# NVIDIA/nvalchemi-toolkit-ops

Measured on AMD Instinct MI355X. Metric: atom-steps/sec (nlist+D3+PME) on 100k-atom PBC box, higher is better.
Workload: dtype f64 (PME) + f32 (D3)

## Files before the change

### nvalchemi-toolkit-ops_amd/csrc/nlist.hip

```cpp
#include <stdlib.h>

#include "binsort.h"
#include "common.h"

namespace {

#define NL_PRUNE_R 8
#ifndef NL_TILE
#define NL_TILE 1024
#endif
#ifndef NL_TILE_F64
#define NL_TILE_F64 768
#endif
#ifndef NL_TILED_WAVES
#define NL_TILED_WAVES 0
#endif
#ifndef NL_CCHUNK
#define NL_CCHUNK 64
#endif
#define NL_MAXROWS 96
#define NL_MIXED 0x7fffffff
#define NL_TILED_GRID 1536
static int nl_tiled_grid() {
  static const int g = [] { const char* e = getenv("NVALCHEMIOPS_NL_TILED_GRID"); const int v = e ? atoi(e) : 0; return v > 0 ? v : NL_TILED_GRID; }();
  return g;
}
template <class T> struct NlSys {
  T cell[9];
  T inv[9];
  T origin[3];
  int cpd[3];
  int R[3];
  int pbc[3];
  int nrange[3];
  int cell_off;
  int ncells;
  int tiled;
  int prune;
  signed char dxlim[NL_PRUNE_R + 1][NL_PRUNE_R + 1];
};
struct NlGlobal {
  int total_cells; int any_wrap; int use_tiled; int pad1;
  int work[4];
  int done[4];
};

struct NlLayout {
  size_t sys, glob, natoms, keys_in, keys_out, vals_in, vals_out, wrap, swrap, spos, srk, cell_start, bins, total;
  long long cell_cap;
};

inline long long nl_cell_cap(int N, int B) { return 4ll * N + 8ll * B; }

inline int nl_key_bits(long long cap) {
  int bits = 1;
  while ((1ll << bits) <= cap && bits < 31) ++bits;
  return bits;
}

NlLayout nl_layout(int N, int B, int dtype) {
  NlLayout L;
  size_t o = 0;
  const size_t sysz = dtype == MI_F32 ? sizeof(NlSys<float>) : sizeof(NlSys<double>);
  const size_t esz = dtype == MI_F32 ? 4 : 8;
  L.cell_cap = nl_cell_cap(N, B);
  auto take = [&](size_t bytes) { size_t at = o; o += mi_align(bytes); return at; };
  L.sys = take(sysz * (size_t)B);
  L.glob = take(sizeof(NlGlobal));
  L.natoms = take(sizeof(int) * (size_t)B);
  L.keys_in = take(sizeof(int) * (size_t)N);
  L.keys_out = take(sizeof(int) * (size_t)N);
  L.vals_in = take(sizeof(int) * (size_t)N);
  L.vals_out = take(sizeof(int) * (size_t)N);
  L.wrap = take(8 * (size_t)N);
  L.swrap = take(8 * (size_t)N);
  L.spos = take(4 * esz * (size_t)N);
  L.srk = take(sizeof(float) * (size_t)N);
  L.cell_start = take(sizeof(int) * (size_t)(L.cell_cap + 2));
  L.bins = take(sizeof(int) * bs_scratch_ints(L.cell_cap + 2));
  L.total = o;
  return L;
}

__device__ __forceinline__ float4 pack4(float x, float y, float z, int idx) { return make_float4(x, y, z, __int_as_float(idx)); }
__device__ __forceinline__ double4 pack4(double x, double y, double z, int idx) { return make_double4(x, y, z, (double)idx); }
__device__ __forceinline__ int idx_of(const float4& v) { return __float_as_int(v.w); }
__device__ __forceinline__ int idx_of(const double4& v) { return (int)v.w; }

__global__ void nl_count_atoms_kernel(const int* __restrict__ batch_idx, int N, int* __restrict__ natoms) {
  const int i = blockIdx.x * blockDim.x + threadIdx.x;
  const bool in = i < N;
  const int s = in ? batch_idx[i] : -1;
  const int s0 = __shfl(s, 0, MI_WAVE);
  const unsigned long long same = __ballot(in && s == s0);
  if ((threadIdx.x & (MI_WAVE - 1)) == 0 && s0 >= 0) atomicAdd(&natoms[s0], __popcll(same));
  if (in && s != s0) atomicAdd(&natoms[s], 1);
}

template <class T>
__device__ void nl_describe_system(const T* __restrict__ cell, const uint8_t* __restrict__ pbc, const int* __restrict__ natoms, int N, T cutoff,
                                   const T* __restrict__ origin, int s, NlSys<T>& S) {
  for (int k = 0; k < 9; ++k) S.cell[k] = cell[9 * (size_t)s + k];
  for (int k = 0; k < 3; ++k) S.origin[k] = origin ? origin[3 * (size_t)s + k] : T(0);
  inverse3(S.cell, S.inv);
  const T* a = S.cell;
  double det = (double)a[0] * ((double)a[4] * a[8] - (double)a[5] * a[7]) - (double)a[1] * ((double)a[3] * a[8] - (double)a[5] * a[6]) +
               (double)a[2] * ((double)a[3] * a[7] - (double)a[4] * a[6]);
  double vol = fabs(det);
  int ns = natoms ? natoms[s] : N;
  double rc = (double)cutoff;
  double apc = vol > 0 ? (double)ns / vol * rc * rc * rc : 0.0;
#ifndef NL_K2_APC
#define NL_K2_APC 64.0
#endif
  int k = apc < NL_K2_APC ? 1 : (apc < 512.0 ? 2 : 3);
  long long cap = 4ll * ns + 8;
  double face[3];
  for (int d = 0; d < 3; ++d) {
    T col[3] = {S.inv[d], S.inv[3 + d], S.inv[6 + d]};
    T ln = sqrt(col[0] * col[0] + col[1] * col[1] + col[2] * col[2]);
    face[d] = 1.0 / (double)ln;
    S.pbc[d] = pbc[3 * (size_t)s + d] ? 1 : 0;
    double want = face[d] * k / (rc * (1.0 + 2e-6));
    S.cpd[d] = want >= 1048576.0 ? 1048576 : (want >= 1.0 ? (int)want : 1);
    S.nrange[d] = S.pbc[d] ? (int)ceil(ln * cutoff) : 0;
  }
  long long tot = (long long)S.cpd[0] * S.cpd[1] * S.cpd[2];
  while (tot > cap) {
    for (int d = 0; d < 3; ++d) S.cpd[d] = S.cpd[d] / 2 > 1 ? S.cpd[d] / 2 : 1;
    tot = (long long)S.cpd[0] * S.cpd[1] * S.cpd[2];
  }
  for (int d = 0; d < 3; ++d) {
    if (S.cpd[d] == 1 && !S.pbc[d]) S.R[d] = 0;
    else S.R[d] = (int)ceil(rc * S.cpd[d] / face[d] * (1.0 + 1e-6));
  }
  S.ncells = (int)tot;
  S.cell_off = 0;
  S.tiled = ((k >= 2 || apc >= 32.0) && (2 * S.R[1] + 1) * (2 * S.R[2] + 1) <= NL_MAXROWS && (!S.pbc[0] || S.R[0] <= S.cpd[0])) ? 1 : 0;
  const bool ortho = a[1] == T(0) && a[2] == T(0) && a[3] == T(0) && a[5] == T(0) && a[6] == T(0) && a[7] == T(0);
  S.prune = (ortho && S.R[0] <= NL_PRUNE_R && S.R[1] <= NL_PRUNE_R && S.R[2] <= NL_PRUNE_R) ? 1 : 0;
}

template <class T>
__global__ __launch_bounds__(256) void nl_setup_kernel(const T* __restrict__ cell, const uint8_t* __restrict__ pbc, const int* __restrict__ natoms, int N,
                                int B, T cutoff, const T* __restrict__ origin, NlSys<T>* __restrict__ sys, NlGlobal* __restrict__ glob,
                                int table_blocks, int4* __restrict__ zero, long long zero_words, int* __restrict__ pk_flag,
                                int* __restrict__ cn_hdr, float cn_scale) {
  constexpr int NE = (NL_PRUNE_R + 1) * (NL_PRUNE_R + 1);
  if (pk_flag && blockIdx.x == 0 && threadIdx.x == 0) *pk_flag = 0;
  if (cn_hdr && blockIdx.x == 0) {
    if (threadIdx.x == 0) { cn_hdr[0] = 0; cn_hdr[1] = 0; cn_hdr[2] = __float_as_int((float)cutoff); cn_hdr[3] = __float_as_int(cn_scale); }
    if (threadIdx.x < MI_CN_SLOTS) reinterpret_cast<unsigned long long*>(cn_hdr)[MI_CN_SLOT_OFFSET_U64 + threadIdx.x] = 0ull;
  }
  if ((int)blockIdx.x > table_blocks) {
    const long long zb = (long long)blockIdx.x - table_blocks - 1, nzb = (long long)gridDim.x - table_blocks - 1;
    for (long long k = zb * blockDim.x + threadIdx.x; k < zero_words; k += nzb * blockDim.x) zero[k] = make_int4(0, 0, 0, 0);
    return;
  }
  if (blockIdx.x > 0) {
    const int t = ((int)blockIdx.x - 1) * blockDim.x + threadIdx.x;
    if (t >= B * NE) return;
    const int s = t / NE, az = (t - s * NE) / (NL_PRUNE_R + 1), ay = t - s * NE - az * (NL_PRUNE_R + 1);
    NlSys<T> S;
    nl_describe_system<T>(cell, pbc, natoms, N, cutoff, origin, s, S);
    if (!S.prune) return;
    const double rc = (double)cutoff;
    double w[3];
    for (int d = 0; d < 3; ++d) {
      const double ln = fabs((double)S.inv[4 * d]);
      w[d] = (S.pbc[d] && ln > 0.0) ? (1.0 / ln) / S.cpd[d] : 0.0;
    }
    const double gz = (az > 1 ? az - 1 : 0) * w[2], gy = (ay > 1 ? ay - 1 : 0) * w[1];
    const double rem = rc * rc - gz * gz - gy * gy;
    int lim;
    if (rem < -1e-6 * rc * rc) lim = -1;
    else if (w[0] > 0.0) { lim = (int)(sqrt(rem > 0.0 ? rem : 0.0) / w[0] * (1.0 + 1e-6)) + 1; if (lim > S.R[0]) lim = S.R[0]; }
    else lim = S.R[0];
    sys[s].dxlim[az][ay] = (signed char)lim;
    return;
  }
  for (int s = threadIdx.x; s < B; s += blockDim.x) {
    NlSys<T> S;
    nl_describe_system<T>(cell, pbc, natoms, N, cutoff, origin, s, S);
    NlSys<T>* dst = sys + s;
    for (int k = 0; k < 9; ++k) { dst->cell[k] = S.cell[k]; dst->inv[k] = S.inv[k]; }
    for (int k = 0; k < 3; ++k) { dst->origin[k] = S.origin[k]; dst->cpd[k] = S.cpd[k]; dst->R[k] = S.R[k]; dst->pbc[k] = S.pbc[k]; dst->nrange[k] = S.nrange[k]; }
    dst->cell_off = 0; dst->ncells = S.ncells; dst->tiled = S.tiled; dst->prune = S.prune;
  }
  __syncthreads();
  __shared__ int wave_tot[4];
  __shared__ int carry_sh, tiled_sh;
  if (threadIdx.x == 0) { carry_sh = 0; tiled_sh = 1; }
  __syncthreads();
  const int lane = threadIdx.x & (MI_WAVE - 1), wave = threadIdx.x / MI_WAVE;
  for (int s0 = 0; s0 < B; s0 += blockDim.x) {
    const int s = s0 + threadIdx.x;
    const int x = s < B ? sys[s].ncells : 0;
    if (s < B && !sys[s].tiled) tiled_sh = 0;
    int inc = x;
#pragma unroll
    for (int o = 1; o < MI_WAVE; o <<= 1) { const int up = __shfl_up(inc, o, MI_WAVE); if (lane >= o) inc += up; }
    if (lane == MI_WAVE - 1) wave_tot[wave] = inc;
    __syncthreads();
    int woff = carry_sh;
    for (int w = 0; w < 4; ++w) woff += (w < wave) ? wave_tot[w] : 0;
    if (s < B) sys[s].cell_off = woff + inc - x;
    __syncthreads();
    if (threadIdx.x == blockDim.x - 1) carry_sh = woff + inc;
    __syncthreads();
  }
  if (threadIdx.x == 0) {
    glob->total_cells = carry_sh;
    glob->any_wrap = 0;
    glob->use_tiled = tiled_sh;
    for (int k = 0; k < 4; ++k) { glob->work[k] = 0; glob->done[k] = 0; }
  }
}

template <class T>
__global__ void nl_assign_kernel(const T* __restrict__ pos, const int* __restrict__ batch_idx, int N, const NlSys<T>* __restrict__ sys,
                                 int* __restrict__ keys, int* __restrict__ count, short4* __restrict__ wrap, NlGlobal* __restrict__ glob) {
  int i = blockIdx.x * blockDim.x + threadIdx.x;
  const bool in = i < N;
  int key = 0;
  if (in) {
    const int s = batch_idx ? batch_idx[i] : 0;
    const NlSys<T>& S = sys[s];
    T p[3] = {pos[3 * (size_t)i] - S.origin[0], pos[3 * (size_t)i + 1] - S.origin[1], pos[3 * (size_t)i + 2] - S.origin[2]}, frac[3];
    rowvec_mat3(p, S.inv, frac);
    int c[3], w[3];
#pragma unroll
    for (int d = 0; d < 3; ++d) {
      int v = (int)floor(frac[d] * (T)S.cpd[d]);
      if (S.pbc[d]) floor_divmod(v, S.cpd[d], w[d], c[d]);
      else { w[d] = 0; c[d] = v < 0 ? 0 : (v >= S.cpd[d] ? S.cpd[d] - 1 : v); }
    }
    key = S.cell_off + c[0] + S.cpd[0] * (c[1] + S.cpd[1] * c[2]);
    keys[i] = key;
    wrap[i] = make_short4((short)w[0], (short)w[1], (short)w[2], 0);
    if (w[0] | w[1] | w[2]) glob->any_wrap = 1;
  }
  bs_wave_add<false>(count, key, in);
}

struct NlCnBuild { const int* numbers; const float* rcov; int nz; float K; float* srk; unsigned long long* slots; const void* cell; int n_cell; const int* batch_idx; };
template <class T>
__global__ void nl_rank_gather_kernel(const T* __restrict__ pos, const int* __restrict__ ids, const int* __restrict__ keys,
                                      const int* __restrict__ cell_start, const short4* __restrict__ wrap, int N,
                                      typename Vec4<T>::type* __restrict__ spos, short4* __restrict__ swrap, int* __restrict__ keys_sorted,
                                      NlCnBuild C) {
  int p = blockIdx.x * blockDim.x + threadIdx.x;
  unsigned long long h = 0;
  if (p < N) {
    const int i = ids[p];
    const int key = keys[i];
    const int b = cell_start[key], e = cell_start[key + 1];
    int rank = 0;
    for (int q = b; q < e; ++q) rank += ids[q] < i ? 1 : 0;
    const int dst = b + rank;
    const T x = pos[3 * (size_t)i], y = pos[3 * (size_t)i + 1], z = pos[3 * (size_t)i + 2];
    spos[dst] = pack4(x, y, z, i);
    swrap[dst] = wrap[i];
    keys_sorted[dst] = key;
    if (C.srk) {
      const float rk = mi_cn_rk(C.numbers[i], C.nz, C.rcov, C.K);
      C.srk[dst] = rk;
      h = mi_cn_atom_hash<T>(i, C.batch_idx ? C.batch_idx[i] : 0, x, y, z, rk);
    }
  }
  if (C.srk) {
    if (p < C.n_cell) h += mi_cn_cell_hash<T>(p, reinterpret_cast<const T*>(C.cell)[p]);
    if (p == 0) h += mi_cn_scale_hash(C.K);
    mi_cn_slot_add(C.slots, p / MI_WAVE, h);
  }
}

struct NlInt3 { int a, b, c; };

template <bool NT = true>
__device__ __forceinline__ void wave_fill(int* __restrict__ dst, long long begin, long long end, int value, int lane) {
  long long n = end - begin;
  if (n <= 0) return;
  int* p = dst + begin;
  int head = (int)(((16 - ((uintptr_t)p & 15)) & 15) >> 2);
  if (head > n) head = (int)n;
  if (lane < head) p[lane] = value;
  long long body = (n - head) >> 2;
  int4* p4 = reinterpret_cast<int4*>(p + head);
  typedef int nl_i4 __attribute__((ext_vector_type(4)));
  const nl_i4 w4 = {value, value, value, value};
  for (long long t = lane; t < body; t += MI_WAVE) {
    if constexpr (NT) __builtin_nontemporal_store(w4, reinterpret_cast<nl_i4*>(p4 + t));
    else *reinterpret_cast<nl_i4*>(p4 + t) = w4;
  }
  long long done = head + (body << 2);
  if (done + lane < n) p[done + lane] = value;
}

__device__ __noinline__ void nl_prefix_runs(int* run_pre, int n, int lane) {
  int carry = 0;
  if (lane == 0) run_pre[0] = 0;
  for (int r0 = 0; r0 < n; r0 += MI_WAVE) {
    const int r = r0 + lane;
    int inc = r < n ? run_pre[r + 1] : 0;
#pragma unroll
    for (int o = 1; o < MI_WAVE; o <<= 1) { const int up = __shfl_up(inc, o, MI_WAVE); if (lane >= o) inc += up; }
    if (r < n) run_pre[r + 1] = carry + inc;
    carry += __shfl(inc, MI_WAVE - 1, MI_WAVE);
  }
}

__device__ __forceinline__ long long nl_uniform64(long long v) {
  const unsigned lo = __builtin_amdgcn_readfirstlane((unsigned)v), hi = __builtin_amdgcn_readfirstlane((unsigned)((unsigned long long)v >> 32));
  return (long long)(((unsigned long long)hi << 32) | lo);
}

__device__ __forceinline__ float nl_uni(float x) { return __int_as_float(__builtin_amdgcn_readfirstlane(__float_as_int(x))); }
__device__ __forceinline__ double nl_uni(double x) { return __longlong_as_double(nl_uniform64(__double_as_longlong(x))); }

template <class T> struct NlSecond { T rc2; int* nm; int* nsh; int* num; int M; };
struct NlPacked { unsigned* words; int* flag; };
struct NlCn { const float* rk; float* cn; int* flag; float K; };
__device__ __forceinline__ float nl_cn_term(float d2, float rki, float rkj, float K) {
  const float rinv = __builtin_amdgcn_rsqf(d2);
  const float t = fmaf(-(rki + rkj), rinv, K);
  return __builtin_amdgcn_rcpf(1.0f + __builtin_amdgcn_exp2f(t));
}
#define NL_PK_PAD 0xffffffffu
#ifndef NL_PREZERO_SHIFTS
#define NL_PREZERO_SHIFTS 1
#endif
#ifndef NL_PREZERO_NT
#define NL_PREZERO_NT 1
#endif
#define NL_PK_ZERO_SHIFT 0x54000000u
__device__ __forceinline__ unsigned nl_pk_code(int Sx, int Sy, int Sz, bool& bad) {
  const unsigned cx = (unsigned)(Sx + 1), cy = (unsigned)(Sy + 1), cz = (unsigned)(Sz + 1);
  bad = (cx > 2u) | (cy > 2u) | (cz > 2u);
  return ((cx & 3u) << 26) | ((cy & 3u) << 28) | (cz << 30);
}

template <class T>
__device__ __forceinline__ bool nl_pair_hit(T pix, T piy, T piz, int i, T cjx, T cjy, T cjz, int j, int Sx, int Sy, int Sz, const T* cart,
                                            T rc2, bool naive, bool half, int nr0, int nr1, int nr2, T* d2_out = nullptr) {
  T dr0, dr1, dr2;
  bool ok = true;
  if (!naive) {
    dr0 = (cjx - pix) + cart[0];
    dr1 = (cjy - piy) + cart[1];
    dr2 = (cjz - piz) + cart[2];
  } else {
    const bool upper = Sx > 0 || (Sx == 0 && Sy > 0) || (Sx == 0 && Sy == 0 && Sz >= 0);
    if (upper) { dr0 = (cart[0] + cjx) - pix; dr1 = (cart[1] + cjy) - piy; dr2 = (cart[2] + cjz) - piz; }
    else { dr0 = ((-cart[0]) + pix) - cjx; dr1 = ((-cart[1]) + piy) - cjy; dr2 = ((-cart[2]) + piz) - cjz; }
    ok = (Sx <= nr0 && -Sx <= nr0) && (Sy <= nr1 && -Sy <= nr1) && (Sz <= nr2 && -Sz <= nr2);
  }
  const T d2 = dr0 * dr0 + dr1 * dr1 + dr2 * dr2;
  if (d2_out) *d2_out = d2;
  const bool zeroS = (Sx | Sy | Sz) == 0;
  bool hit = ok && (d2 < rc2) && !(j == i && zeroS);
  if (half && hit) {
    const bool pos_shift = Sx > 0 || (Sx == 0 && Sy > 0) || (Sx == 0 && Sy == 0 && Sz > 0);
    hit = pos_shift || (zeroS && j > i);
  }
  return hit;
}

template <class T, int MODE, bool FAST, bool DUAL = false, bool CNF = false>
#if NL_TILED_WAVES > 0
__global__ __launch_bounds__(256) __attribute__((amdgpu_waves_per_eu(NL_TILED_WAVES, NL_TILED_WAVES))) void nl_query_tiled_kernel(
#else
__global__ __launch_bounds__(256) __attribute__((amdgpu_waves_per_eu((CNF && sizeof(T) == 4) ? 5 : 1, (CNF && sizeof(T) == 4) ? 5 : 8))) void nl_query_tiled_kernel(
#endif
    const typename Vec4<T>::type* __restrict__ spos, const short4* __restrict__ swrap, const int* __restrict__ cell_start,
    const NlSys<T>* __restrict__ sys, const NlGlobal* __restrict__ glob, int B, T rc2, int flags, int* __restrict__ nm,
    int* __restrict__ nsh, int* __restrict__ num, int M, int fill_value, const int* __restrict__ ptr, int* __restrict__ list_ij,
    int* __restrict__ list_sh, long long P, NlSecond<T> D, NlPacked K, NlCn CN = NlCn{nullptr, nullptr, nullptr, 0.0f}) {
  static_assert(!DUAL || (MODE == MI_NL_MODE_MATRIX && !FAST), "the dual-cutoff sweep is instantiated for the general matrix kernel only");
  static_assert(!CNF || (MODE == MI_NL_MODE_MATRIX && FAST && !DUAL), "coordination numbers ride with the plain full-list matrix search");
  constexpr int TILE = sizeof(T) == 8 ? NL_TILE_F64 : NL_TILE;
  if (!glob->use_tiled) return;
  if (!DUAL && FAST != ((flags & (MI_NL_HALF_FILL | MI_NL_NAIVE_EXPR)) == 0)) return;
  __shared__ float trk[CNF ? TILE : 1], cen_rk[CNF ? NL_CCHUNK : 1];
  __shared__ double ccn[CNF ? NL_CCHUNK : 1];
  __shared__ int ccnt2[DUAL ? NL_CCHUNK : 1];
  __shared__ T tx[TILE], ty[TILE], tz[TILE];
  __shared__ int tj[TILE];
  __shared__ short tsx[CNF ? 1 : TILE], tsy[CNF ? 1 : TILE], tsz[CNF ? 1 : TILE];
  __shared__ int tsp[CNF ? TILE : 1];
  __shared__ int run_beg[3 * NL_MAXROWS], run_pre[3 * NL_MAXROWS + 1], run_cs[3 * NL_MAXROWS];
  __shared__ int ccnt[NL_CCHUNK];
  __shared__ T cen_x[NL_CCHUNK], cen_y[NL_CCHUNK], cen_z[NL_CCHUNK];
  __shared__ int cen_i[NL_CCHUNK];
  __shared__ short4 cen_w[NL_CCHUNK];
  __shared__ int grp_run[TILE / MI_WAVE];
  __shared__ int grp_shift[TILE / MI_WAVE];
  __shared__ int u_store[CNF ? 1 : 9 * NL_MAXROWS];
  static_assert(sizeof(T) * TILE >= sizeof(int) * 9 * NL_MAXROWS, "the run table must fit the x array of a tile");
  int* const u_beg = CNF ? reinterpret_cast<int*>(tx) : u_store;
  int* const u_len = u_beg + 3 * NL_MAXROWS;
  int* const u_cs = u_beg + 6 * NL_MAXROWS;
  const int tid = threadIdx.x, lane = tid & (MI_WAVE - 1), wave = tid / MI_WAVE;
  const int total_cells = glob->total_cells;
  const bool anyw = glob->any_wrap != 0;
  const bool half = (flags & MI_NL_HALF_FILL) != 0, naive = (flags & MI_NL_NAIVE_EXPR) != 0;
  const unsigned long long lt = (1ull << lane) - 1ull;
  __shared__ int next_cell;
  NlGlobal* gw = const_cast<NlGlobal*>(glob);
  for (;;) {
    __syncthreads();
    if (tid == 0) next_cell = atomicAdd(&gw->work[MODE], 1);
    __syncthreads();
    const int c = next_cell;
    if (c >= total_cells) break;
    const int c_beg = cell_start[c], n_c = cell_start[c + 1] - c_beg;
    if (n_c == 0) continue;
    int s = 0;
    {
      int lo = 0, hi = B - 1;
      while (lo < hi) { const int mid = (lo + hi + 1) >> 1; if (sys[mid].cell_off <= c) lo = mid; else hi = mid - 1; }
      s = lo;
    }
    const NlSys<T>* S = sys + s;
    const int nx = S->cpd[0], ny = S->cpd[1], nz = S->cpd[2];
    const int Rx = S->R[0], Ry = S->R[1], Rz = S->R[2];
    const bool pbx = S->pbc[0] != 0, pby = S->pbc[1] != 0, pbz = S->pbc[2] != 0;
    const int coff = S->cell_off;
    const int nr0 = S->nrange[0], nr1 = S->nrange[1], nr2 = S->nrange[2];
    T cm[9];
#pragma unroll
    for (int k = 0; k < 9; ++k) cm[k] = S->cell[k];
    const int local = c - coff;
    const int cx = local % nx, cyz = local / nx, cy = cyz % ny, cz = cyz / ny;
    const int nyr = 2 * Ry + 1, nrows = (2 * Rz + 1) * nyr;
    __syncthreads();
    if (tid < nrows) {
      const int dzr = tid / nyr, dz = dzr - Rz, dy = tid - dzr * nyr - Ry;
      const int tzc = cz + dz, tyc = cy + dy;
      bool ok = (pbz || (tzc >= 0 && tzc < nz)) && (pby || (tyc >= 0 && tyc < ny));
      int csz = 0, wz = tzc, csy = 0, wy = tyc;
      if (ok) {
        while (wz < 0) { wz += nz; --csz; }
        while (wz >= nz) { wz -= nz; ++csz; }
        while (wy < 0) { wy += ny; --csy; }
        while (wy >= ny) { wy -= ny; ++csy; }
      }
      int dxm = Rx;
      if (S->prune) { dxm = S->dxlim[dz < 0 ? -dz : dz][dy < 0 ? -dy : dy]; ok = ok && dxm >= 0; }
      int xlo = cx - dxm, xhi = cx + dxm;
      if (!pbx) { xlo = xlo < 0 ? 0 : xlo; xhi = xhi > nx - 1 ? nx - 1 : xhi; }
      const int rowbase = coff + nx * (wy + ny * wz);
      for (int g = 0; g < 3; ++g) {
        const int img0 = (g - 1) * nx;
        const int xa = (xlo > img0 ? xlo : img0), xb = (xhi < img0 + nx - 1 ? xhi : img0 + nx - 1);
        int b = 0, len = 0;
        if (ok && xa <= xb && (pbx || g == 1)) { b = cell_start[rowbase + xa - img0]; len = cell_start[rowbase + xb - img0 + 1] - b; }
        u_beg[3 * tid + g] = b;
        u_len[3 * tid + g] = len;
        u_cs[3 * tid + g] = ((g - 1) & 0x3ff) | ((csy & 0x3ff) << 10) | ((csz & 0x3ff) << 20);
      }
    }
    __syncthreads();
    for (int r = tid; r < 3 * nrows; r += 256) {
      const int key = u_cs[r];
      int rank = 0;
      for (int q = 0; q < 3 * nrows; ++q) {
        const int kq = u_cs[q];
        rank += ((unsigned)kq < (unsigned)key) || (kq == key && q < r);
      }
      run_beg[rank] = u_beg[r];
      run_pre[rank + 1] = u_len[r];
      run_cs[rank] = key;
    }
    __syncthreads();
    if (wave == 0) nl_prefix_runs(run_pre, 3 * nrows, lane);
    __syncthreads();
    const int nruns = 3 * nrows, total = run_pre[nruns];
    for (int cbase = 0; cbase < n_c; cbase += NL_CCHUNK) {
      const int cend = (cbase + NL_CCHUNK < n_c) ? cbase + NL_CCHUNK : n_c;
      if (tid < NL_CCHUNK) {
        ccnt[tid] = 0;
        if (DUAL) ccnt2[tid] = 0;
        if (cbase + tid < cend) {
          const auto cr = spos[c_beg + cbase + tid];
          cen_x[tid] = cr.x; cen_y[tid] = cr.y; cen_z[tid] = cr.z;
          cen_i[tid] = idx_of(cr);
          cen_w[tid] = anyw ? swrap[c_beg + cbase + tid] : make_short4(0, 0, 0, 0);
          if (CNF) { cen_rk[tid] = CN.rk[c_beg + cbase + tid]; ccn[tid] = 0.0; }
        }
      }
      for (int tile0 = 0; tile0 < total; tile0 += TILE) {
        const int tile_n = (total - tile0 < TILE) ? total - tile0 : TILE;
        __syncthreads();
        if (tid < TILE / MI_WAVE && tile0 + tid * MI_WAVE < total) {
          const int v = tile0 + tid * MI_WAVE;
          int lo = 0, hi = nruns - 1;
          while (lo < hi) { const int mid = (lo + hi + 1) >> 1; if (run_pre[mid] <= v) lo = mid; else hi = mid - 1; }
          grp_run[tid] = lo;
        }
        __syncthreads();
        for (int t = tid; t < tile_n; t += 256) {
          const int v = tile0 + t;
          int lo = grp_run[t / MI_WAVE];
          while (lo + 1 < nruns && run_pre[lo + 1] <= v) ++lo;
          const int q = run_beg[lo] + (v - run_pre[lo]);
          const auto rec = spos[q];
          tx[t] = rec.x; ty[t] = rec.y; tz[t] = rec.z;
          tj[t] = idx_of(rec);
          if (CNF) trk[t] = CN.rk[q];
          const int cs = run_cs[lo];
          int sx = (cs << 22) >> 22, sy = (cs << 12) >> 22, sz = (cs << 2) >> 22;
          if (anyw) {
            const short4 wj = swrap[q];
            if (pbx) sx -= wj.x;
            if (pby) sy -= wj.y;
            if (pbz) sz -= wj.z;
          }
          if (CNF) tsp[t] = (sx & 0x3ff) | ((sy & 0x3ff) << 10) | ((sz & 0x3ff) << 20);
          else { tsx[t] = (short)sx; tsy[t] = (short)sy; tsz[t] = (short)sz; }
          const int cs0 = __builtin_amdgcn_readfirstlane(cs);
          const bool same = __all(cs == cs0) && !anyw;
          if (lane == 0) grp_shift[t / MI_WAVE] = same ? cs0 : NL_MIXED;
        }
        __syncthreads();
        constexpr int NC = 2;
        for (int ci0 = cbase + wave; ci0 < cend; ci0 += 4 * NC) {
          T ccx[NC], ccy[NC], ccz[NC];
          int ii[NC], cap_row[NC], cnt[NC], cnt2[NC];
          float rki[NC], cnp[NC];
          long long out_base[NC];
          short4 wi[NC];
          const int nc = (cend - ci0 + 3) / 4 < NC ? (cend - ci0 + 3) / 4 : NC;
#pragma unroll
          for (int u = 0; u < NC; ++u) {
            const bool live = u < nc;
            const int ci = live ? ci0 + 4 * u : ci0;
            ccx[u] = live ? cen_x[ci - cbase] : (T)NAN; ccy[u] = cen_y[ci - cbase]; ccz[u] = cen_z[ci - cbase];
            if (CNF) { ccx[u] = nl_uni(ccx[u]); ccy[u] = nl_uni(ccy[u]); ccz[u] = nl_uni(ccz[u]); }
            ii[u] = __builtin_amdgcn_readfirstlane(cen_i[ci - cbase]);
            wi[u] = cen_w[ci - cbase];
            if (MODE == MI_NL_MODE_CSR) { out_base[u] = ptr[ii[u]]; cap_row[u] = ptr[ii[u] + 1] - ptr[ii[u]]; }
            else { out_base[u] = (long long)ii[u] * M; cap_row[u] = M; }
            cnt[u] = ccnt[ci - cbase];
            cnt2[u] = DUAL ? ccnt2[ci - cbase] : 0;
            if (CNF) { rki[u] = nl_uni(cen_rk[ci - cbase]); cnp[u] = 0.0f; }
          }
          const bool ortho = S->prune != 0;
          int* row_j[NC];
          NlInt3* row_s[NC];
          unsigned* row_p[NC];
#pragma unroll
          for (int u = 0; u < NC; ++u) {
            const long long ob = nl_uniform64(out_base[u]);
            row_p[u] = (MODE == MI_NL_MODE_MATRIX && !DUAL && K.words) ? K.words + ob : nullptr;
            if (MODE == MI_NL_MODE_MATRIX) { row_j[u] = nm + ob; row_s[u] = nsh ? reinterpret_cast<NlInt3*>(nsh) + ob : nullptr; }
            else if (MODE == MI_NL_MODE_CSR) { row_j[u] = list_ij + P + ob; row_s[u] = list_sh ? reinterpret_cast<NlInt3*>(list_sh) + ob : nullptr; }
            else { row_j[u] = nullptr; row_s[u] = nullptr; }
          }
          constexpr bool PREZERO = NL_PREZERO_SHIFTS && MODE == MI_NL_MODE_MATRIX && !DUAL;
          const bool prezero = PREZERO && nsh && !(flags & MI_NL_NO_PAD);
          if (PREZERO && prezero && tile0 == 0) {
#pragma unroll
            for (int u = 0; u < NC; ++u)
              if (u < nc) wave_fill<NL_PREZERO_NT != 0>(nsh, out_base[u] * 3, (out_base[u] + M) * 3, 0, lane);
            asm volatile("s_waitcnt vmcnt(0)" ::: "memory");
          }
          auto emit_m = [&](int u, unsigned long long mask, bool hit, int j, int Sx, int Sy, int Sz, unsigned code, bool zero_shift = false) {
            if (MODE == MI_NL_MODE_COUNT) { cnt[u] += __popcll(mask); return; }
            if (mask) {
              const unsigned slot = __builtin_amdgcn_mbcnt_hi((unsigned)(mask >> 32), __builtin_amdgcn_mbcnt_lo((unsigned)mask, (unsigned)cnt[u]));
              if (hit && slot < (unsigned)cap_row[u]) {
                *reinterpret_cast<int*>(reinterpret_cast<char*>(row_j[u]) + slot * 4u) = j;
                if (row_s[u] && !(PREZERO && prezero && zero_shift))
                  *reinterpret_cast<NlInt3*>(reinterpret_cast<char*>(row_s[u]) + __umul24(slot, 12u)) = NlInt3{Sx, Sy, Sz};
                if (MODE == MI_NL_MODE_MATRIX && !DUAL && row_p[u]) *reinterpret_cast<unsigned*>(reinterpret_cast<char*>(row_p[u]) + slot * 4u) = (unsigned)j | code;
              }
              cnt[u] += __popcll(mask);
            }
          };
          auto emit = [&](int u, bool hit, int j, int Sx, int Sy, int Sz, unsigned code) { emit_m(u, __builtin_amdgcn_ballot_w64(hit), hit, j, Sx, Sy, Sz, code); };
          struct Cand { int j, tt, zg; T x, y, z; };
          auto fetch = [&](int t0) {
            Cand c;
            const int t = t0 + lane;
            const bool in = t < tile_n;
            c.tt = in ? t : 0;
            c.j = tj[c.tt];
            c.x = in ? tx[c.tt] : (T)NAN;
            c.y = ty[c.tt]; c.z = tz[c.tt];
            c.zg = grp_shift[(t0 < tile_n ? t0 : 0) / MI_WAVE];
            return c;
          };
          Cand nxt = fetch(0);
          for (int t0 = 0; t0 < tile_n; t0 += MI_WAVE) {
            const Cand cur = nxt;
            nxt = fetch(t0 + MI_WAVE);
            const int j = cur.j, tt = cur.tt;
            const float rkj = CNF ? trk[tt] : 0.0f;
            const T cjx = cur.x, cjy = cur.y, cjz = cur.z;
            const int gs = __builtin_amdgcn_readfirstlane(cur.zg);
            if (FAST && gs == 0) {
#pragma unroll
              for (int u = 0; u < NC; ++u) {
                const T dr0 = cjx - ccx[u], dr1 = cjy - ccy[u], dr2 = cjz - ccz[u];
                const T d2 = dr0 * dr0 + dr1 * dr1 + dr2 * dr2;
                const bool in = d2 < rc2, other = j != ii[u];
                if (CNF) cnp[u] += (in & other & ((float)d2 >= 1e-24f)) ? nl_cn_term((float)d2, rki[u], rkj, CN.K) : 0.0f;
                emit_m(u, __builtin_amdgcn_ballot_w64(in) & __builtin_amdgcn_ballot_w64(other), in & other, j, 0, 0, 0, NL_PK_ZERO_SHIFT, true);
              }
            } else if (FAST && gs != NL_MIXED) {
              const int Sx = (gs << 22) >> 22, Sy = (gs << 12) >> 22, Sz = (gs << 2) >> 22;
              T cart[3];
              if (ortho) { cart[0] = cm[0] * (T)Sx; cart[1] = cm[4] * (T)Sy; cart[2] = cm[8] * (T)Sz; }
              else { const T fs[3] = {(T)Sx, (T)Sy, (T)Sz}; rowvec_mat3(fs, cm, cart); }
              bool bad;
              const unsigned code = nl_pk_code(Sx, Sy, Sz, bad);
#pragma unroll
              for (int u = 0; u < NC; ++u) {
                const T dr0 = (cjx - ccx[u]) + cart[0], dr1 = (cjy - ccy[u]) + cart[1], dr2 = (cjz - ccz[u]) + cart[2];
                const T d2 = dr0 * dr0 + dr1 * dr1 + dr2 * dr2;
                const bool h = d2 < rc2;
                if (CNF) cnp[u] += (h & ((float)d2 >= 1e-24f)) ? nl_cn_term((float)d2, rki[u], rkj, CN.K) : 0.0f;
                if (MODE == MI_NL_MODE_MATRIX && bad && row_p[u] && h) *K.flag = 1;
                emit(u, h, j, Sx, Sy, Sz, code);
              }
            } else {
              int Sx0, Sy0, Sz0;
              if (CNF) { const int w = tsp[tt]; Sx0 = (w << 22) >> 22; Sy0 = (w << 12) >> 22; Sz0 = (w << 2) >> 22; }
              else { Sx0 = tsx[tt]; Sy0 = tsy[tt]; Sz0 = tsz[tt]; }
#pragma unroll
              for (int u = 0; u < NC; ++u) {
                int Sx = Sx0, Sy = Sy0, Sz = Sz0;
                if (anyw) { if (pbx) Sx += wi[u].x; if (pby) Sy += wi[u].y; if (pbz) Sz += wi[u].z; }
                T cart[3];
                if (ortho) { cart[0] = cm[0] * (T)Sx; cart[1] = cm[4] * (T)Sy; cart[2] = cm[8] * (T)Sz; }
                else { const T fs[3] = {(T)Sx, (T)Sy, (T)Sz}; rowvec_mat3(fs, cm, cart); }
                bool h;
                if (FAST) {
                  const T dr0 = (cjx - ccx[u]) + cart[0], dr1 = (cjy - ccy[u]) + cart[1], dr2 = (cjz - ccz[u]) + cart[2];
                  const T d2 = dr0 * dr0 + dr1 * dr1 + dr2 * dr2;
                  h = (d2 < rc2) & !((j == ii[u]) & ((Sx | Sy | Sz) == 0));
                  if (CNF) cnp[u] += (h & ((float)d2 >= 1e-24f)) ? nl_cn_term((float)d2, rki[u], rkj, CN.K) : 0.0f;
                } else {
                  T d2;
                  h = nl_pair_hit<T>(ccx[u], ccy[u], ccz[u], ii[u], cjx, cjy, cjz, j, Sx, Sy, Sz, cart, rc2, naive, half, nr0, nr1, nr2, &d2);
                  if (DUAL) {
                    const bool h2 = h && (d2 < D.rc2);
                    const unsigned long long m2 = __ballot(h2);
                    if (m2) {
                      const int slot = cnt2[u] + __popcll(m2 & lt);
                      if (h2 && slot < D.M) {
                        const long long o = (long long)ii[u] * D.M + slot;
                        D.nm[o] = j;
                        if (D.nsh) reinterpret_cast<NlInt3*>(D.nsh)[o] = NlInt3{Sx, Sy, Sz};
                      }
                      cnt2[u] += __popcll(m2);
                    }
                  }
                }
                bool bad;
                const unsigned code = nl_pk_code(Sx, Sy, Sz, bad);
                if (MODE == MI_NL_MODE_MATRIX && !DUAL && bad && row_p[u] && h) *K.flag = 1;
                emit(u, h, j, Sx, Sy, Sz, code);
              }
            }
          }
          if (CNF) {
#pragma unroll
            for (int u = 0; u < NC; ++u) {
              const double part = wave_sum((double)cnp[u]);
              if (lane == 0 && u < nc) ccn[ci0 + 4 * u - cbase] += part;
            }
          }
          if (lane == 0) {
#pragma unroll
            for (int u = 0; u < NC; ++u) if (u < nc) { ccnt[ci0 + 4 * u - cbase] = cnt[u]; if (DUAL) ccnt2[ci0 + 4 * u - cbase] = cnt2[u]; }
          }
        }
      }
      __syncthreads();
      for (int ci = cbase + wave; ci < cend; ci += 4) {
        const int i = __builtin_amdgcn_readfirstlane(cen_i[ci - cbase]);
        const int cnt = ccnt[ci - cbase];
        if (MODE != MI_NL_MODE_CSR) { if (lane == 0) num[i] = cnt; }
        if (CNF && lane == 0) {
          CN.cn[i] = (float)ccn[ci - cbase];
          if (cnt > M) *CN.flag = 1;
        }
        if (MODE == MI_NL_MODE_CSR) {
          const long long rb = ptr[i];
          const int room = ptr[i + 1] - ptr[i];
          wave_fill(list_ij, rb, rb + (cnt < room ? cnt : room), i, lane);
        }
        if (MODE == MI_NL_MODE_MATRIX && !(flags & MI_NL_NO_PAD)) {
          const long long out_base = (long long)i * M;
          const int used = cnt < M ? cnt : M;
          wave_fill(nm, out_base + used, out_base + M, fill_value, lane);
          if (nsh && !(NL_PREZERO_SHIFTS && !DUAL)) wave_fill(nsh, (out_base + used) * 3, (out_base + M) * 3, 0, lane);
          if (!DUAL && K.words) wave_fill(reinterpret_cast<int*>(K.words), out_base + used, out_base + M, (int)NL_PK_PAD, lane);
        }
        if (DUAL) {
          const int c2 = ccnt2[ci - cbase];
          if (lane == 0) D.num[i] = c2;
          if (!(flags & MI_NL_NO_PAD)) {
            const long long ob = (long long)i * D.M;
            const int used = c2 < D.M ? c2 : D.M;
            wave_fill(D.nm, ob + used, ob + D.M, fill_value, lane);
            if (D.nsh) wave_fill(D.nsh, (ob + used) * 3, (ob + D.M) * 3, 0, lane);
          }
        }
// ... 763 lines not shown
```

Before: 31.61 million.

## Pack tiled nlist LDS into one struct and shrink CN tile for occupancy

Groups all shared-memory arrays of the tiled neighbor-list kernel into a single struct and always aliases the run table onto the start of the tile arrays, dropping the separate u_store buffer for non-CN variants. It adds a smaller tile size for the CN-summing fp32 variant (768 instead of 1024) so five of those blocks plus one fp64 block fit a CU's LDS together. The aim is higher occupancy and co-residency, in exchange for more tile iterations in the CN search.

```diff
diff --git a/nvalchemi-toolkit-ops_amd/csrc/nlist.hip b/nvalchemi-toolkit-ops_amd/csrc/nlist.hip
--- a/nvalchemi-toolkit-ops_amd/csrc/nlist.hip
+++ b/nvalchemi-toolkit-ops_amd/csrc/nlist.hip
@@ -8,6 +8,9 @@
 #define NL_PRUNE_R 8
 #ifndef NL_TILE
 #define NL_TILE 1024
+#endif
+#ifndef NL_TILE_CN
+#define NL_TILE_CN 768
 #endif
 #ifndef NL_TILE_F64
 #define NL_TILE_F64 768
@@ -366,6 +369,28 @@
   return hit;
 }
 
+template <class T, bool DUAL, bool CNF> struct NlTiledLds {
+  static constexpr int TILE = sizeof(T) == 8 ? NL_TILE_F64 : (CNF ? NL_TILE_CN : NL_TILE);
+  T tx[TILE], ty[TILE], tz[TILE];
+  int tj[TILE];
+  float trk[CNF ? TILE : 1];
+  int tsp[CNF ? TILE : 1];
+  short tsx[CNF ? 1 : TILE], tsy[CNF ? 1 : TILE], tsz[CNF ? 1 : TILE];
+  int run_beg[3 * NL_MAXROWS], run_pre[3 * NL_MAXROWS + 1], run_cs[3 * NL_MAXROWS];
+  int grp_run[TILE / MI_WAVE];
+  int grp_shift[TILE / MI_WAVE];
+  double ccn[CNF ? NL_CCHUNK : 1];
+  T cen_x[NL_CCHUNK], cen_y[NL_CCHUNK], cen_z[NL_CCHUNK];
+  short4 cen_w[NL_CCHUNK];
+  int cen_i[NL_CCHUNK];
+  float cen_rk[CNF ? NL_CCHUNK : 1];
+  int ccnt[NL_CCHUNK];
+  int ccnt2[DUAL ? NL_CCHUNK : 1];
+  int next_cell;
+};
+static_assert(5 * sizeof(NlTiledLds<float, false, true>) + sizeof(NlTiledLds<double, false, false>) <= 160 * 1024,
+              "five blocks of the CN-summing fp32 search and one block of the fp64 search must fit the LDS of a CU together");
+
 template <class T, int MODE, bool FAST, bool DUAL = false, bool CNF = false>
 #if NL_TILED_WAVES > 0
 __global__ __launch_bounds__(256) __attribute__((amdgpu_waves_per_eu(NL_TILED_WAVES, NL_TILED_WAVES))) void nl_query_tiled_kernel(
@@ -378,26 +403,19 @@
     int* __restrict__ list_sh, long long P, NlSecond<T> D, NlPacked K, NlCn CN = NlCn{nullptr, nullptr, nullptr, 0.0f}) {
   static_assert(!DUAL || (MODE == MI_NL_MODE_MATRIX && !FAST), "the dual-cutoff sweep is instantiated for the general matrix kernel only");
   static_assert(!CNF || (MODE == MI_NL_MODE_MATRIX && FAST && !DUAL), "coordination numbers ride with the plain full-list matrix search");
-  constexpr int TILE = sizeof(T) == 8 ? NL_TILE_F64 : NL_TILE;
+  using Lds = NlTiledLds<T, DUAL, CNF>;
+  constexpr int TILE = Lds::TILE;
+  static_assert(TILE % MI_WAVE == 0, "tiles are whole 64-candidate groups");
   if (!glob->use_tiled) return;
   if (!DUAL && FAST != ((flags & (MI_NL_HALF_FILL | MI_NL_NAIVE_EXPR)) == 0)) return;
-  __shared__ float trk[CNF ? TILE : 1], cen_rk[CNF ? NL_CCHUNK : 1];
-  __shared__ double ccn[CNF ? NL_CCHUNK : 1];
-  __shared__ int ccnt2[DUAL ? NL_CCHUNK : 1];
-  __shared__ T tx[TILE], ty[TILE], tz[TILE];
-  __shared__ int tj[TILE];
-  __shared__ short tsx[CNF ? 1 : TILE], tsy[CNF ? 1 : TILE], tsz[CNF ? 1 : TILE];
-  __shared__ int tsp[CNF ? TILE : 1];
-  __shared__ int run_beg[3 * NL_MAXROWS], run_pre[3 * NL_MAXROWS + 1], run_cs[3 * NL_MAXROWS];
-  __shared__ int ccnt[NL_CCHUNK];
-  __shared__ T cen_x[NL_CCHUNK], cen_y[NL_CCHUNK], cen_z[NL_CCHUNK];
-  __shared__ int cen_i[NL_CCHUNK];
-  __shared__ short4 cen_w[NL_CCHUNK];
-  __shared__ int grp_run[TILE / MI_WAVE];
-  __shared__ int grp_shift[TILE / MI_WAVE];
-  __shared__ int u_store[CNF ? 1 : 9 * NL_MAXROWS];
-  static_assert(sizeof(T) * TILE >= sizeof(int) * 9 * NL_MAXROWS, "the run table must fit the x array of a tile");
-  int* const u_beg = CNF ? reinterpret_cast<int*>(tx) : u_store;
+  __shared__ Lds lds;
+  auto& tx = lds.tx; auto& ty = lds.ty; auto& tz = lds.tz; auto& tj = lds.tj; auto& trk = lds.trk;
+  auto& tsp = lds.tsp; auto& tsx = lds.tsx; auto& tsy = lds.tsy; auto& tsz = lds.tsz;
+  auto& run_beg = lds.run_beg; auto& run_pre = lds.run_pre; auto& run_cs = lds.run_cs; auto& grp_run = lds.grp_run; auto& grp_shift = lds.grp_shift;
+  auto& ccn = lds.ccn; auto& cen_x = lds.cen_x; auto& cen_y = lds.cen_y; auto& cen_z = lds.cen_z; auto& cen_w = lds.cen_w; auto& cen_i = lds.cen_i;
+  auto& cen_rk = lds.cen_rk; auto& ccnt = lds.ccnt; auto& ccnt2 = lds.ccnt2; auto& next_cell = lds.next_cell;
+  static_assert(offsetof(Lds, trk) >= sizeof(int) * 9 * NL_MAXROWS, "the run table must fit the position and index arrays of a tile");
+  int* const u_beg = reinterpret_cast<int*>(&lds);
   int* const u_len = u_beg + 3 * NL_MAXROWS;
   int* const u_cs = u_beg + 6 * NL_MAXROWS;
   const int tid = threadIdx.x, lane = tid & (MI_WAVE - 1), wave = tid / MI_WAVE;
@@ -405,7 +423,6 @@
   const bool anyw = glob->any_wrap != 0;
   const bool half = (flags & MI_NL_HALF_FILL) != 0, naive = (flags & MI_NL_NAIVE_EXPR) != 0;
   const unsigned long long lt = (1ull << lane) - 1ull;
-  __shared__ int next_cell;
   NlGlobal* gw = const_cast<NlGlobal*>(glob);
   for (;;) {
     __syncthreads();
```

After: 31.59 million. No clear change (-0.1%).
